# kyshu11027/financial-chatbot-llm

Hardware: AMD Instinct MI355X
Metric: chat turns/sec + p50 TTFT, Llama-3-8B RAG agent at 1/2/4/8 MI355X (higher is better)
Workload: dtype bf16

## Files before the change

financial_chatbot_llm_amd/csrc/kernels/gemm_splitk.hip:

```cpp
#include "common.h"

#include <utility>

typedef __attribute__((address_space(3))) void lds_void_t;
typedef __attribute__((address_space(1))) const void gbl_void_t;

namespace {

template <int N>
__device__ __forceinline__ void vmcnt_barrier() {
  static_assert(N >= 0 && N < 64, "vmcnt range");
  asm volatile("s_waitcnt vmcnt(%0)\n\ts_barrier" ::"n"(N) : "memory");
}

union Frag {
  uint4 u;
  bf16x8 v;
};

enum { SK_SLAB = 0, SK_SILU = 1, SK_BF16 = 2, SK_SAMPLE = 3, SK_SAMPLE_LP = 4 };

struct SkSample {
  const float* temps;
  const unsigned long long* seeds;
  float* pv;
  int* pi;
  int pstride, voff, vvalid;
};

__device__ __forceinline__ int xswz(int r, int c) { return c ^ (r & 7) ^ ((r >> 3) & 1); }

template <int NF, int MT, int KB = 150, int MAXB = 8, int BKM = 1>
struct Ring {
  static constexpr int SBYTES = (NF + MT) * 2 * 1024 * BKM;
  static constexpr int LOADS = (2 * NF + 2 * MT) / 4 * BKM;
  static constexpr int BY_LDS = KB * 1024 / SBYTES;
  static constexpr int BY_VM = 63 / LOADS + 2;
  static constexpr int CAP = MAXB / BKM > 3 ? MAXB / BKM : 3;
  static constexpr int NBUF = BY_LDS < CAP ? (BY_LDS < BY_VM ? BY_LDS : BY_VM) : (CAP < BY_VM ? CAP : BY_VM);
};

template <class F, int... U>
__device__ __forceinline__ void static_for_impl(F&& f, std::integer_sequence<int, U...>) {
  (f(std::integral_constant<int, U>{}), ...);
}
template <int N, class F>
__device__ __forceinline__ void static_for(F&& f) {
  static_for_impl(f, std::make_integer_sequence<int, N>{});
}

template <int LOADS, int MAXY>
__device__ __forceinline__ void wait_stage(int younger) {
  if constexpr (MAXY <= 0) {
    vmcnt_barrier<0>();
  } else {
    if (younger >= MAXY) vmcnt_barrier<MAXY * LOADS>();
    else wait_stage<LOADS, MAXY - 1>(younger);
  }
}

template <int FW, int TW, int WBYTES, bool WROW>
__device__ __forceinline__ void stage_mma(const char* __restrict__ base, f32x4 (&acc)[FW][TW], int wa, int wb,
                                          int lane, int g, int col) {
#pragma unroll
  for (int kk = 0; kk < 2; ++kk) {
    Frag wf[FW], xf[TW];
#pragma unroll
    for (int f = 0; f < FW; ++f) {
      if constexpr (WROW) {
        const int r = (wa * FW + f) * 16 + col;
        wf[f].u = *reinterpret_cast<const uint4*>(base + r * 128 + xswz(r, 4 * kk + g) * 16);
      } else {
        wf[f].u = *reinterpret_cast<const uint4*>(base + ((wa * FW + f) * 2 + kk) * 1024 + lane * 16);
      }
    }
#pragma unroll
    for (int t = 0; t < TW; ++t) {
      const int r = (wb * TW + t) * 16 + col;
      xf[t].u = *reinterpret_cast<const uint4*>(base + WBYTES + r * 128 + xswz(r, 4 * kk + g) * 16);
    }
#pragma unroll
    for (int f = 0; f < FW; ++f)
#pragma unroll
      for (int t = 0; t < TW; ++t)
        acc[f][t] = __builtin_amdgcn_mfma_f32_16x16x32_bf16(wf[f].v, xf[t].v, acc[f][t], 0, 0, 0);
  }
}

template <int NF, int MT, int WA, int EPI = SK_SLAB, bool WROW = false, int RKB = 150, int MAXB = 8, int BKM = 1>
__global__ void __launch_bounds__(256, 1) splitk_gemm_kernel(const bf16* __restrict__ X, int ldx,
                                                             const bf16* __restrict__ Wt, int K,
                                                             float* __restrict__ P, int M, int N, int S,
                                                             bf16* __restrict__ Y = nullptr, int ldy = 0,
                                                             SkSample sa = SkSample{}) {
  constexpr bool SILU = EPI == SK_SILU;
  constexpr int WB = 4 / WA;
  constexpr int FW = NF / WA;
  constexpr int TW = MT / WB;
  static_assert(NF % WA == 0 && MT % WB == 0, "wave split");
  static_assert(!SILU || FW % 2 == 0, "SiLU epilogue needs (gate, up) row-group pairs per wave");
  constexpr int NBUF = Ring<NF, MT, RKB, MAXB, BKM>::NBUF;
  static_assert(NBUF >= 3, "ring too shallow");
  constexpr int WBYTES = NF * 2 * 1024;
  constexpr int XBYTES = MT * 2 * 1024;
  constexpr int SBYTES = WBYTES + XBYTES;
  constexpr int PIECES = (2 * NF + 2 * MT);
  static_assert(PIECES % 4 == 0, "pieces must split evenly over 4 waves");
  constexpr int LOADS = PIECES / 4;
  constexpr int SLOT = BKM * SBYTES;
  __shared__ __attribute__((aligned(1024))) char smem[NBUF * SLOT];

  const int lane = threadIdx.x & 63, w = threadIdx.x >> 6, g = lane >> 4, col = lane & 15;
  const int s = blockIdx.x % S, tile = blockIdx.x / S;
  const int Mtot = M, m0 = blockIdx.y * 16 * MT;
  M = min(Mtot - m0, 16 * MT);
  X += (long)m0 * ldx;
  if constexpr (EPI == SK_SILU || EPI == SK_BF16) Y += (long)m0 * ldy;
  PENNY_DASSERT(M > 0 && ((EPI != SK_SAMPLE && EPI != SK_SAMPLE_LP) || gridDim.y == 1));
  PENNY_DASSERT((tile + 1) * 16 * NF <= N && K % (64 * BKM * S) == 0);
  const int n0 = tile * 16 * NF;
  const int kc = K / S, k0 = s * kc;
  const int nst = kc / (64 * BKM);
  const int ksteps = K / 32;
  const int wa = w / WB, wb = w % WB;

  const char* src[LOADS];
  int dst[LOADS];
  long step[LOADS];
#pragma unroll
  for (int i = 0; i < LOADS; ++i) {
    const int q = w * LOADS + i;
    if (q < 2 * NF && WROW) {
      const int r = q * 8 + (lane >> 3);
      const int c = xswz(r, lane & 7);
      src[i] = reinterpret_cast<const char*>(Wt + (long)(n0 + r) * K + k0 + 8 * c);
      step[i] = 128;
      dst[i] = q * 1024;
    } else if (q < 2 * NF) {
      const int f = q >> 1, kk = q & 1;
      src[i] = reinterpret_cast<const char*>(Wt) +
               (((long)(n0 / 16 + f) * ksteps + k0 / 32 + kk) * 64 + lane) * 16;
      step[i] = 2 * 1024;
      dst[i] = (f * 2 + kk) * 1024;
    } else {
      const int xp = q - 2 * NF;
      const int r = xp * 8 + (lane >> 3);
      const int c = xswz(r, lane & 7);
      const int row = min(r, M - 1);
      src[i] = reinterpret_cast<const char*>(X + (long)row * ldx + k0 + 8 * c);
      step[i] = 128;
      dst[i] = WBYTES + xp * 1024;
    }
  }
  auto stage = [&](int j) {
    char* base = smem + (j % NBUF) * SLOT;
#pragma unroll
    for (int i = 0; i < LOADS; ++i)
#pragma unroll
      for (int u = 0; u < BKM; ++u)
        __builtin_amdgcn_global_load_lds((gbl_void_t*)(src[i] + (j * BKM + u) * step[i]),
                                         (lds_void_t*)(base + u * SBYTES + dst[i]), 16, 0, 0);
  };

  f32x4 acc[FW][TW];
#pragma unroll
  for (int f = 0; f < FW; ++f)
#pragma unroll
    for (int t = 0; t < TW; ++t) acc[f][t] = f32x4{0.f, 0.f, 0.f, 0.f};

#pragma unroll
  for (int j = 0; j < NBUF - 1; ++j)
    if (j < nst) stage(j);

  for (int j = 0; j < nst; ++j) {
    wait_stage<LOADS * BKM, NBUF - 2>(min(NBUF - 2, nst - 1 - j));
    if (j + NBUF - 1 < nst) stage(j + NBUF - 1);
#pragma unroll
    for (int u = 0; u < BKM; ++u)
      stage_mma<FW, TW, WBYTES, WROW>(smem + (j % NBUF) * SLOT + u * SBYTES, acc, wa, wb, lane, g, col);
  }

  if constexpr (SILU) {
#pragma unroll
    for (int t = 0; t < TW; ++t) {
      const int m = (wb * TW + t) * 16 + col;
      if (m >= M) continue;
#pragma unroll
      for (int f = 0; f < FW; f += 2) {
        const int G = n0 / 16 + wa * FW + f;
        bf16x4 o;
#pragma unroll
        for (int r = 0; r < 4; ++r) {
          const float gt = (float)(bf16)acc[f][t][r], up = (float)(bf16)acc[f + 1][t][r];
          o[r] = (bf16)((float)(bf16)(gt / (1.f + __expf(-gt))) * up);
        }
        *reinterpret_cast<bf16x4*>(Y + (long)m * ldy + (G >> 1) * 16 + 4 * g) = o;
      }
    }
    return;
  }
  if constexpr (EPI == SK_BF16) {
#pragma unroll
    for (int t = 0; t < TW; ++t) {
      const int m = (wb * TW + t) * 16 + col;
      if (m >= M) continue;
#pragma unroll
      for (int f = 0; f < FW; ++f) {
        bf16x4 o;
#pragma unroll
        for (int r = 0; r < 4; ++r) o[r] = (bf16)acc[f][t][r];
        *reinterpret_cast<bf16x4*>(Y + (long)m * ldy + n0 + (wa * FW + f) * 16 + 4 * g) = o;
      }
    }
    return;
  }
  if constexpr (EPI == SK_SAMPLE) {
#pragma unroll
    for (int t = 0; t < TW; ++t) {
      const int m = (wb * TW + t) * 16 + col;
      if (m >= M) continue;
      const float temp = sa.temps[m];
      const bool greedy = !(temp > 0.f);
      const float inv_t = greedy ? 1.f : 1.f / temp;
      const unsigned long long seed = sa.seeds[m];
      float bv = -INFINITY;
      int bi = 0x7fffffff;
#pragma unroll
      for (int f = 0; f < FW; ++f)
#pragma unroll
        for (int r = 0; r < 4; ++r) {
          const int loc = n0 + (wa * FW + f) * 16 + 4 * g + r, idx = sa.voff + loc;
          float v = (float)(bf16)acc[f][t][r];
          if (!greedy) v = v * inv_t + gumbel_noise(seed, idx);
          if (loc >= sa.vvalid) v = -INFINITY;
          better(bv, bi, v, idx);
        }
#pragma unroll
      for (int o = 16; o < 64; o <<= 1) {
        const float ov = __shfl_xor(bv, o, 64);
        const int oi = __shfl_xor(bi, o, 64);
        better(bv, bi, ov, oi);
      }
      if (g == 0) {
        const long slot = (long)m * sa.pstride + tile * WA + wa;
        sa.pv[slot] = bv;
        sa.pi[slot] = bi;
      }
    }
    return;
  }
  if constexpr (EPI == SK_SAMPLE_LP) {
    const long plane = (long)Mtot * sa.pstride;
    float* pl = sa.pv + 2 * plane;
    float* pm = pl + plane;
    float* pe = pm + plane;
#pragma unroll
    for (int t = 0; t < TW; ++t) {
      const int m = (wb * TW + t) * 16 + col;
      if (m >= M) continue;
      const float temp = sa.temps[m];
      const bool greedy = !(temp > 0.f);
      const float inv_t = greedy ? 1.f : 1.f / temp;
      const unsigned long long seed = sa.seeds[m];
      const int loc0 = n0 + wa * FW * 16 + 4 * g;
      float bv = -INFINITY, bl = -INFINITY, mx = -INFINITY;
      int bi = 0x7fffffff;
#pragma unroll
      for (int f = 0; f < FW; ++f)
#pragma unroll
        for (int r = 0; r < 4; ++r) {
          const int loc = loc0 + f * 16 + r, idx = sa.voff + loc;
          const float l = (float)(bf16)acc[f][t][r];
          float v = l;
          if (!greedy) v = v * inv_t + gumbel_noise(seed, idx);
          if (loc >= sa.vvalid) v = -INFINITY;
          else mx = fmaxf(mx, l);
          better_lp(bv, bi, bl, v, idx, l);
        }
#pragma unroll
      for (int o = 16; o < 64; o <<= 1) {
        const float ov = __shfl_xor(bv, o, 64);
        const int oi = __shfl_xor(bi, o, 64);
        const float ol = __shfl_xor(bl, o, 64);
        better_lp(bv, bi, bl, ov, oi, ol);
        mx = fmaxf(mx, __shfl_xor(mx, o, 64));
      }
      float se = 0.f;
#pragma unroll
      for (int f = 0; f < FW; ++f)
#pragma unroll
        for (int r = 0; r < 4; ++r)
          if (loc0 + f * 16 + r < sa.vvalid) se += __expf((float)(bf16)acc[f][t][r] - mx);
#pragma unroll
      for (int o = 16; o < 64; o <<= 1) se += __shfl_xor(se, o, 64);
      if (g == 0) {
        const long slot = (long)m * sa.pstride + tile * WA + wa;
        sa.pv[slot] = bv;
        sa.pi[slot] = bi;
        pl[slot] = bl;
        pm[slot] = mx;
        pe[slot] = se;
      }
    }
    return;
  }
  float* ps = P + (long)s * Mtot * N + (long)m0 * N;
#pragma unroll
  for (int t = 0; t < TW; ++t) {
    const int m = (wb * TW + t) * 16 + col;
    if (m >= M) continue;
#pragma unroll
    for (int f = 0; f < FW; ++f) {
      const int n = n0 + (wa * FW + f) * 16 + 4 * g;
      *reinterpret_cast<f32x4*>(ps + (long)m * N + n) = acc[f][t];
    }
  }
}

__global__ void __launch_bounds__(256) splitk_reduce_kernel(const float* __restrict__ P, int S, int M, int N,
                                                            bf16* __restrict__ Y, int ldy,
                                                            const bf16* __restrict__ R, int ldr) {
  const long i8 = (long)blockIdx.x * 256 + threadIdx.x;
  const long total8 = (long)M * N / 8;
  if (i8 >= total8) return;
  const int m = (int)(i8 / (N / 8));
  const int n = (int)(i8 % (N / 8)) * 8;
  float o[8];
  {
    const f32x4* p = reinterpret_cast<const f32x4*>(P + (long)m * N + n);
    const f32x4 a = p[0], b = p[1];
#pragma unroll
    for (int j = 0; j < 4; ++j) o[j] = a[j], o[4 + j] = b[j];
  }
  for (int s = 1; s < S; ++s) {
    const f32x4* p = reinterpret_cast<const f32x4*>(P + ((long)s * M + m) * N + n);
    const f32x4 a = p[0], b = p[1];
#pragma unroll
    for (int j = 0; j < 4; ++j) o[j] += a[j], o[4 + j] += b[j];
  }
  if (R) {
    float r[8];
    unpack8(*reinterpret_cast<const uint4*>(R + (long)m * ldr + n), r);
#pragma unroll
    for (int j = 0; j < 8; ++j) o[j] = (float)(bf16)o[j] + r[j];
  }
  *reinterpret_cast<uint4*>(Y + (long)m * ldy + n) = pack8(o);
}

template <int NF, int MT, int RKB, int MAXB>
constexpr bool pair_fits() {
  return Ring<NF, MT, RKB, MAXB, 2>::NBUF >= 3;
}

constexpr int wave_split(int nf, int mt) { return nf >= 6 || mt <= 2 || (mt > 4 && mt <= 6) ? 2 : 1; }

template <int NF, int MT, int EPI, int MAXB, int WA = wave_split(NF, MT), class... A>
int launch_any(int wrow, bool pair_ok, dim3 grid, hipStream_t st, A... args) {
  const bool rm = wrow & 1;
  if constexpr (pair_fits<NF, MT, 150, MAXB>()) {
    if ((wrow & 2) && pair_ok) {
      if (rm) hipLaunchKernelGGL((splitk_gemm_kernel<NF, MT, WA, EPI, true, 150, MAXB, 2>), grid, dim3(256), 0, st, args...);
      else hipLaunchKernelGGL((splitk_gemm_kernel<NF, MT, WA, EPI, false, 150, MAXB, 2>), grid, dim3(256), 0, st, args...);
      return (int)hipGetLastError();
    }
  }
  if (rm) hipLaunchKernelGGL((splitk_gemm_kernel<NF, MT, WA, EPI, true, 150, MAXB>), grid, dim3(256), 0, st, args...);
  else hipLaunchKernelGGL((splitk_gemm_kernel<NF, MT, WA, EPI, false, 150, MAXB>), grid, dim3(256), 0, st, args...);
  return (int)hipGetLastError();
}

template <int NF, int MT>
int launch(const void* X, int ldx, const void* Wt, int K, float* P, int M, int N, int S, int wrow, hipStream_t st) {
  return launch_any<NF, MT, SK_SLAB, 8>(wrow, (K / S) % 128 == 0, dim3((N / (16 * NF)) * S, (M + 16 * MT - 1) / (16 * MT)), st, (const bf16*)X,
                                            ldx, (const bf16*)Wt, K, P, M, N, S, (bf16*)nullptr, 0, SkSample{});
}

template <int NF, int MT>
int launch_silu(const void* X, int ldx, const void* Wt, int K, void* Y, int ldy, int M, int N, int wrow,
                hipStream_t st) {
  constexpr int WA = NF == 2 ? 1 : wave_split(NF, MT);
  return launch_any<NF, MT, SK_SILU, NF == 2 ? 16 : 8, WA>(wrow, K % 128 == 0, dim3(N / (16 * NF), (M + 16 * MT - 1) / (16 * MT)), st, (const bf16*)X,
                                                          ldx, (const bf16*)Wt, K, (float*)nullptr, M, N, 1, (bf16*)Y,
                                                          ldy, SkSample{});
}

template <int NF, int MT>
int launch_bf16(const void* X, int ldx, const void* Wt, int K, void* Y, int ldy, int M, int N, int wrow,
                hipStream_t st) {
  return launch_any<NF, MT, SK_BF16, 16>(wrow, K % 128 == 0, dim3(N / (16 * NF), (M + 16 * MT - 1) / (16 * MT)), st, (const bf16*)X, ldx,
                                             (const bf16*)Wt, K, (float*)nullptr, M, N, 1, (bf16*)Y, ldy, SkSample{});
}

template <int NF, int MT, int EPI>
int launch_sample(const void* X, int ldx, const void* Wt, int K, int M, int N, int wrow, int ring2, const SkSample& sa,
                  hipStream_t st) {
  constexpr int WA = wave_split(NF, MT);
  const dim3 grid(N / (16 * NF)), block(256);
#define SK_SAMPLE_LAUNCH(WROW_, KB_)                                                                               \
  hipLaunchKernelGGL((splitk_gemm_kernel<NF, MT, WA, EPI, WROW_, KB_, 16>), grid, block, 0, st, (const bf16*)X, ldx, \
// ... 39 lines not shown
  return (int)hipErrorInvalidValue;
}

PENNY_API int penny_splitk_gemm(const void* X, int ldx, const void* Wt, int K, void* P, int M, int N, int S, int nf,
                                int wrow, hipStream_t stream) {
  if (M <= 0) return 0;
  if (M > (1 << 20) || S < 1 || K % (64 * S) || ldx % 8 || (nf != 2 && nf != 4 && nf != 6 && nf != 8) || N % (16 * nf))
    return (int)hipErrorInvalidValue;
  const int mt = min((M + 15) / 16, 16);
  float* p = static_cast<float*>(P);
#define SK_CASE(MT_)                                                             \
  if (mt <= MT_) {                                                               \
    if (nf == 2) return launch<2, MT_>(X, ldx, Wt, K, p, M, N, S, wrow, stream); \
    if (nf == 4) return launch<4, MT_>(X, ldx, Wt, K, p, M, N, S, wrow, stream); \
    if (nf == 6) return launch<6, MT_>(X, ldx, Wt, K, p, M, N, S, wrow, stream); \
    return launch<8, MT_>(X, ldx, Wt, K, p, M, N, S, wrow, stream);              \
  }
  SK_CASE(2) SK_CASE(4) SK_CASE(6) SK_CASE(8) SK_CASE(12) SK_CASE(16)
#undef SK_CASE
  return (int)hipErrorInvalidValue;
}

__global__ void __launch_bounds__(256) splitk_reduce_silu_kernel(const float* __restrict__ P, int S, int M, int N,
                                                                 bf16* __restrict__ Y, int ldy) {
  const int F = N / 2;
  const long i8 = (long)blockIdx.x * 256 + threadIdx.x;
  const long total8 = (long)M * F / 8;
  if (i8 >= total8) return;
  const int m = (int)(i8 / (F / 8));
  const int f = (int)(i8 % (F / 8)) * 8;
  const int ng = (f >> 4) * 32 + (f & 15);
  float gt[8], up[8];
#pragma unroll
  for (int j = 0; j < 8; ++j) gt[j] = up[j] = 0.f;
  for (int s = 0; s < S; ++s) {
    const f32x4* pg = reinterpret_cast<const f32x4*>(P + ((long)s * M + m) * N + ng);
    const f32x4* pu = reinterpret_cast<const f32x4*>(P + ((long)s * M + m) * N + ng + 16);
    const f32x4 g0 = pg[0], g1 = pg[1], u0 = pu[0], u1 = pu[1];
#pragma unroll
    for (int j = 0; j < 4; ++j) gt[j] += g0[j], gt[4 + j] += g1[j], up[j] += u0[j], up[4 + j] += u1[j];
  }
  float o[8];
#pragma unroll
  for (int j = 0; j < 8; ++j) {
    const float gb = (float)(bf16)gt[j], ub = (float)(bf16)up[j];
    o[j] = (float)(bf16)(gb / (1.f + __expf(-gb))) * ub;
  }
  *reinterpret_cast<uint4*>(Y + (long)m * ldy + f) = pack8(o);
}

PENNY_API int penny_splitk_reduce_silu(const void* P, int S, int M, int N, void* Y, int ldy, hipStream_t stream) {
  if (M <= 0) return 0;
  if (N % 32 || ldy % 8 || S < 1) return (int)hipErrorInvalidValue;
  const long total8 = (long)M * (N / 2) / 8;
  hipLaunchKernelGGL(splitk_reduce_silu_kernel, dim3((unsigned)((total8 + 255) / 256)), dim3(256), 0, stream,
                     (const float*)P, S, M, N, (bf16*)Y, ldy);
  return (int)hipGetLastError();
}

PENNY_API int penny_splitk_reduce(const void* P, int S, int M, int N, void* Y, int ldy, const void* R, int ldr,
                                  hipStream_t stream) {
  if (M <= 0) return 0;
  if (N % 8 || ldy % 8 || (R && ldr % 8)) return (int)hipErrorInvalidValue;
  const long total8 = (long)M * N / 8;
  hipLaunchKernelGGL(splitk_reduce_kernel, dim3((unsigned)((total8 + 255) / 256)), dim3(256), 0, stream,
                     (const float*)P, S, M, N, (bf16*)Y, ldy, (const bf16*)R, ldr);
  return (int)hipGetLastError();
}

PENNY_API int penny_splitk_gemm_bf16(const void* X, int ldx, const void* Wt, int K, void* Y, int ldy, int M, int N,
                                     int nf, int wrow, hipStream_t stream) {
  if (M <= 0) return 0;
  if (M > (1 << 20) || K % 64 || ldx % 8 || ldy % 4 || (nf != 2 && nf != 4 && nf != 8) || N % (16 * nf))
    return (int)hipErrorInvalidValue;
  const int mt = min((M + 15) / 16, 16);
#define BF_CASE(MT_)                                                                    \
  if (mt <= MT_) {                                                                      \
    if (nf == 2) return launch_bf16<2, MT_>(X, ldx, Wt, K, Y, ldy, M, N, wrow, stream); \
    if (nf == 4) return launch_bf16<4, MT_>(X, ldx, Wt, K, Y, ldy, M, N, wrow, stream); \
    return launch_bf16<8, MT_>(X, ldx, Wt, K, Y, ldy, M, N, wrow, stream);              \
  }
  BF_CASE(2) BF_CASE(4) BF_CASE(6) BF_CASE(8) BF_CASE(12) BF_CASE(16)
#undef BF_CASE
  return (int)hipErrorInvalidValue;
}

extern "C" int penny_lm_sample_logprob_final(const float* pv, const int* pi, const float* pl, const float* pm,
                                             const float* ps, int P, int M, int* out, float* logprob,
                                             hipStream_t stream);

template <int EPI, class Merge>
static int stream_sample(const void* X, int ldx, const void* W, int K, int M, int Vpad, int vvalid, int voff,
                         const float* temps, const unsigned long long* seeds, void* workspace, int nf, int wrow,
                         int ring2, hipStream_t stream, Merge merge) {
  if (M > 128 || (nf != 4 && nf != 8) || Vpad % (16 * nf) || vvalid <= 0 || vvalid > Vpad || voff < 0 || K % 64 ||
      ldx % 8 || !temps || !seeds || !workspace)
    return (int)hipErrorInvalidValue;
  const int tiles = Vpad / (16 * nf), mt = (M + 15) / 16;
  const int pstride = tiles * wave_split(nf, mt);
  float* pv = static_cast<float*>(workspace);
  int* pi = reinterpret_cast<int*>(pv + (long)M * pstride);
  const SkSample sa{temps, seeds, pv, pi, pstride, voff, vvalid};
  int rc;
#define LS_CASE(MT_)                                                                            \
  if (mt <= MT_) {                                                                              \
    if (nf == 4) rc = launch_sample<4, MT_, EPI>(X, ldx, W, K, M, Vpad, wrow, ring2, sa, stream); \
    else rc = launch_sample<8, MT_, EPI>(X, ldx, W, K, M, Vpad, wrow, ring2, sa, stream);         \
  } else
  LS_CASE(2) LS_CASE(4) LS_CASE(6) LS_CASE(8)
  return (int)hipErrorInvalidValue;
#undef LS_CASE
  if (rc) return rc;
  return merge(pv, pi, pstride);
}

PENNY_API int penny_lm_head_stream_sample(const void* X, int ldx, const void* W, int K, int M, int Vpad, int vvalid,
                                          int voff, const float* temps, const unsigned long long* seeds,
                                          void* workspace, int* out, int* pairs, int nf, int wrow, int ring2,
                                          hipStream_t stream) {
  if (M <= 0) return 0;
  if (!out && !pairs) return (int)hipErrorInvalidValue;
  return stream_sample<SK_SAMPLE>(X, ldx, W, K, M, Vpad, vvalid, voff, temps, seeds, workspace, nf, wrow, ring2,
                                  stream, [=](const float* pv, const int* pi, int P) {
                                    return penny_lm_sample_final(pv, pi, P, M, out, pairs, stream);
                                  });
}

PENNY_API int penny_lm_head_stream_sample_logprob(const void* X, int ldx, const void* W, int K, int M, int Vpad,
                                                  int vvalid, int voff, const float* temps,
                                                  const unsigned long long* seeds, void* workspace, int* out,
                                                  float* logprob, int nf, int wrow, int ring2, hipStream_t stream) {
  if (M <= 0) return 0;
  if (!out || !logprob) return (int)hipErrorInvalidValue;
  return stream_sample<SK_SAMPLE_LP>(X, ldx, W, K, M, Vpad, vvalid, voff, temps, seeds, workspace, nf, wrow, ring2,
                                     stream, [=](const float* pv, const int* pi, int P) {
                                       const long plane = (long)M * P;
                                       return penny_lm_sample_logprob_final(pv, pi, pv + 2 * plane, pv + 3 * plane,
                                                                            pv + 4 * plane, P, M, out, logprob,
                                                                            stream);
                                     });
}
```

financial_chatbot_llm_amd/ops/_native.py:

```python
from __future__ import annotations

import ctypes
import os
import threading
from typing import Optional

import torch

_LOCK = threading.Lock()
_LIB: Optional[ctypes.CDLL] = None
_ERR: Optional[str] = None

c_int, c_long, c_float, c_void_p = ctypes.c_int, ctypes.c_long, ctypes.c_float, ctypes.c_void_p
P = c_void_p

_SIGS = {
    "penny_rmsnorm": [P, P, P, P, c_int, c_int, c_float, c_int, P],
    "penny_rmsnorm_slabs": [P, c_int, P, P, P, c_int, c_int, c_float, c_int, P],
    "penny_layernorm": [P, P, P, P, P, c_int, c_int, c_float, c_int, P],
    "penny_silu_mul": [P, P, c_int, c_int, c_int, P],
    "penny_skinny_gemm": [P, c_int, P, c_int, P, c_int, P, c_int, c_int, c_int, c_int, c_int, c_int, P],
    "penny_splitk_gemm": [P, c_int, P, c_int, P, c_int, c_int, c_int, c_int, c_int, P],
    "penny_splitk_reduce": [P, c_int, c_int, c_int, P, c_int, P, c_int, P],
    "penny_splitk_gemm_bf16": [P, c_int, P, c_int, P, c_int, c_int, c_int, c_int, c_int, P],
    "penny_lm_head_stream_sample": [P, c_int, P, c_int, c_int, c_int, c_int, c_int, P, P, P, P, P, c_int, c_int,
                                    c_int, P],
    "penny_lm_sample_final": [P, P, c_int, c_int, P, P, P],
    "penny_gateup_silu_gemm": [P, c_int, P, c_int, P, c_int, c_int, c_int, c_int, c_int, P],
    "penny_gemm_prefill": [P, c_int, P, c_int, P, c_int, P, c_int, c_int, c_int, c_int, c_int,
                           P, c_long, P, c_int, c_int, P],
    "penny_gemm_prefill_wt": [P, c_int, P, c_int, P, c_int, P, c_int, c_int, c_int, c_int, c_int,
                              P, c_long, P, c_int, c_int, P],
    "penny_gemm_prefill_qkv_rope": [P, c_int, P, c_int, c_int, P, P, P, P, P, P, c_int, c_int,
                                    c_float, P, c_long, P, c_int, c_int, P],
    "penny_gemm_mid_variant": [c_int],
    "penny_gemm_mid": [P, c_int, P, c_int, P, c_int, P, c_int, c_int, c_int, c_int, c_int, P],
    "penny_gemm_prefill_ablate": [P, c_int, P, c_int, P, c_int, c_int, c_int, c_int, P],
    "penny_moe_gemm_prefill_fp8": [P, c_int, P, P, P, P, P, P, P, c_int, c_int, c_int, c_int, c_int, c_int, P],
    "penny_probe_mfma_scale": [P, P, P, P, P, c_int, P],
    "penny_moe_gemm_prefill_fp8_mx": [P, c_int, P, P, P, P, P, P, P, c_int, c_int, c_int, c_int, c_int, c_int, P,
                                      c_int, P],
    "penny_gelu": [P, c_long, P],
    "penny_embedding": [P, P, P, c_int, c_int, c_int, c_int, P],
    "penny_rope_qk": [P, P, P, P, c_int, c_int, c_int, c_int, P],
    "penny_rope_kv_write": [P, P, P, P, P, P, P, c_int, c_int, c_int, c_int, c_int, P],
    "penny_rope_kv_write_slabs": [P, c_int, P, P, P, P, P, P, c_int, c_int, c_int, c_int, c_int, P],
    "penny_rope_kv_write_fp8": [P, P, P, P, P, P, P, P, c_int, c_int, c_int, c_int, c_int, P],
    "penny_rope_kv_write_slabs_fp8": [P, c_int, P, P, P, P, P, P, P, c_int, c_int, c_int, c_int, c_int, P],
    "penny_kv_dequant_fp8": [P, P, P, c_long, c_int, c_int, P],
    "penny_attention_decode_fp8": [P, P, P, P, P, P, P, P, P, c_int, c_int, c_int, c_int, c_int, c_int, c_int,
                                   c_float, c_int, P, c_int, c_int, P, P],
    "penny_attention_prefill_fp8": [P, P, P, P, P, P, P, c_int, c_int, c_int, c_int, c_int, c_int, c_float, c_int, P,
                                    P, c_int, P, P],
    "penny_attention_prefill_lean_fp8": [P, P, P, P, P, P, P, c_int, c_int, c_int, c_int, c_float, c_int, P, P,
                                         c_int, P, c_int, P, P, P, P],
    "penny_attention_prefill": [P, P, P, P, P, P, P, c_int, c_int, c_int, c_int, c_int, c_int, c_float, c_int, P, P,
                                c_int, P],
    "penny_attention_prefill_variant": [c_int],
    "penny_gemm_prefill_set_group": [c_int],
    "penny_attention_prefill_lean": [P, P, P, P, P, P, P, c_int, c_int, c_int, c_int, c_float, c_int, P, P, c_int, P,
                                     c_int, P, P, P],
    "penny_splitk_reduce_silu": [P, c_int, c_int, c_int, P, c_int, P],
    "penny_attention_decode": [P, P, P, P, P, P, P, P, P, c_int, c_int, c_int, c_int, c_int, c_int, c_int, c_int,
                               c_float, c_int, P, c_int, c_int, P],
    "penny_sample": [P, c_int, c_long, P, P, P, P, P, P, c_int, c_int, P],
    "penny_sample_fsm": [P, c_int, c_long, P, P, P, P, P, P, c_int, c_int, P, P, P, c_int, c_int, P, P, P, c_int, P,
                         c_int, P],
    "penny_fsm_build_masks": [P, P, P, P, P, c_int, c_int, c_int, c_int, c_int, c_int, P],
    "penny_pen_reset": [P, c_int, c_int, c_int, c_int, P, c_int, P],
    "penny_pen_add": [P, c_int, c_int, c_int, P, c_int, P],
    "penny_pen_apply": [P, c_int, c_long, P, P, P, P, P, P, c_int, c_int, P, c_int, c_int, P],
    "penny_lm_head_sample": [P, c_int, P, c_int, c_int, c_int, P, P, P, P, P],
    "penny_lm_head_sample_shard": [P, c_int, P, c_int, c_int, c_int, c_int, c_int, P, P, P, P, P],
    "penny_lm_head_logprob": [P, c_int, P, c_int, c_int, c_int, c_int, c_int, P, P, P, P, P],
    "penny_lm_head_sample_logprob": [P, c_int, P, c_int, c_int, c_int, c_int, c_int, P, P, P, P, P, P],
    "penny_lm_head_stream_sample_logprob": [P, c_int, P, c_int, c_int, c_int, c_int, c_int, P, P, P, P, P, c_int,
                                            c_int, c_int, P],
    "penny_lm_sample_logprob_final": [P, P, P, P, P, c_int, c_int, P, P, P],
    "penny_token_logprob": [P, c_int, c_long, P, P, c_int, c_int, P],
    "penny_sample_shard": [P, c_int, c_long, P, P, P, P, c_int, c_int, c_int, P],
    "penny_topk_topp_threshold": [P, c_int, c_long, P, P, P, P, c_int, c_int, P],
    "penny_moe_route": [P, c_int, c_int, c_int, P, P, P, P, P],
    "penny_moe_route_quant": [P, c_int, P, c_int, c_int, c_int, c_int, P, P, P, P, P, P, P, P, P],
    "penny_quant_rows_fp8": [P, c_int, c_int, c_int, P, P, P],
    "penny_silu_quant_rows_fp8": [P, c_int, c_int, P, P, P],
    "penny_moe_gemm_fp8": [P, P, P, P, P, P, P, P, c_int, c_int, c_int, c_int, c_int, P],
    "penny_moe_combine": [P, P, c_int, c_int, c_int, P, P],
    "penny_moe_combine_weighted": [P, P, P, c_int, c_int, c_int, P, P],
    "penny_filtered_topk": [P, P, P, c_long, c_int, P, P, P, P, c_int, c_int, P, P, P, c_int, P, P, P, P],
}


def lib_path() -> str:
    if os.environ.get("PENNY_KERNEL_LIB"):
        return os.environ["PENNY_KERNEL_LIB"]
    from .._build import kernel_lib
    return kernel_lib(os.environ.get("PENNY_KERNEL_DEBUG") == "1")


def load(build_if_missing: bool = True) -> ctypes.CDLL:
    global _LIB, _ERR
    if _LIB is not None:
        return _LIB
    with _LOCK:
        if _LIB is not None:
            return _LIB
        path = lib_path()
# ... 50 lines not shown
```

financial_chatbot_llm_amd/ops/gemm.py:

```python
from __future__ import annotations

import os
from typing import Dict, List, Optional, Tuple, Union

import torch
import torch.nn.functional as F

from . import _native as N
from .activation import silu_mul

EPI = {None: 0, "silu": 1, "residual": 2}
MAX_SKINNY_M = 64
TUNING: Dict[Tuple[int, int], Tuple[int, int]] = {(6144, 4096): (2, 4), (4096, 4096): (1, 4)}
SKINNY_MAX_M: Dict[Tuple[int, int], int] = {(6144, 4096): 16, (4096, 4096): 32}


def _config(N_: int, K: int, epilogue: Optional[str]) -> Tuple[int, int]:
    if (N_, K) in TUNING:
        return TUNING[(N_, K)]
    ntf = 2
    wgs = N_ // (16 * ntf)
    nw = 8 if wgs < 512 else 4
    if K % (nw * 128):
        nw = 4 if K % 512 == 0 else 1
    return ntf, nw


def tile_weight(w: torch.Tensor) -> torch.Tensor:
    N_, K = w.shape
    assert N_ % 16 == 0 and K % 32 == 0
    return w.view(N_ // 16, 16, K // 32, 4, 8).permute(0, 2, 3, 1, 4).reshape(N_ // 16, K // 32, 64, 8).contiguous()


def skinny_ok(x: torch.Tensor, w: torch.Tensor, epilogue: Optional[str] = None,
              wt: Optional[torch.Tensor] = None) -> bool:
    M, K = x.shape
    N_ = w.shape[0]
    if wt is None or not N.use_native(x) or M > MAX_SKINNY_M or os.environ.get("PENNY_SKINNY", "1") == "0":
        return False
    if M > SKINNY_MAX_M.get((N_, K), MAX_SKINNY_M if (N_, K) in TUNING else 0):
        return False
    ntf, nw = _config(N_, K, epilogue)
    return N_ % (16 * ntf) == 0 and K % (nw * 128) == 0 and x.stride(1) == 1 and w.is_contiguous()


def linear(x: torch.Tensor, w: torch.Tensor, epilogue: Optional[str] = None,
           residual: Optional[torch.Tensor] = None, wt: Optional[torch.Tensor] = None,
           slabs: bool = False, fuse_residual: Optional[torch.Tensor] = None) -> Union[torch.Tensor, "Slabs",
                                                                                     "ResidualSum"]:
    M, K = x.shape
    N_ = w.shape[0]
    if M > 256 and prefill_ok(x, w) and epilogue in (None, "silu", "residual"):
        fr = fuse_residual is not None and epilogue is None and residual is None
        c = prefill_choice(M, N_, K, epilogue, slabs and residual is None, fused_residual=fr)
        if c.startswith("K"):
            return splitk_bf16(x, w, N_, int(c[1:]))
        if c == "R":
            prefill_gemm(x, w, "residual", residual=fuse_residual, out=fuse_residual)
            return ResidualSum(fuse_residual)
        if c == "hip":
            return prefill_gemm(x, w, epilogue, residual=residual)
        if c.startswith("S"):
            return Slabs(prefill_gemm(x, w, "slabs", int(c[1:])))
        if c.startswith("M"):
            return mid_linear(x, w, int(c[1:]), epilogue, slabs and residual is None, residual)
    src = wt if wt is not None else (w if w.is_contiguous() else None)
    rowmajor = wt is None
    if slabs and src is not None and epilogue is None and residual is None:
        cfg = splitk_config(M, N_, K) if N.use_native(x) and x.stride(1) == 1 and x.stride(0) % 8 == 0 else None
        if cfg is not None:
            return Slabs(splitk_partials(x, src, N_, *cfg, rowmajor=rowmajor))
    if not slabs and epilogue is None and residual is None and N.use_native(x) and x.stride(1) == 1 \
            and x.stride(0) % 8 == 0:
        cfg = bf16_config(M, N_, K)
        if cfg is not None:
            S, nf, rm = cfg
            rm = rm or wt is None
            ww = w if rm else wt
            if S == 1:
                return splitk_bf16(x, ww, N_, nf, rowmajor=rm)
            return splitk_reduce(splitk_partials(x, ww, N_, S, nf, rowmajor=rm))
    if epilogue == "silu" and src is not None and residual is None:
        ok = N.use_native(x) and x.stride(1) == 1 and x.stride(0) % 8 == 0
        nf = gateup_config(M, N_, K) if ok else None
        if nf is not None:
            return gateup_silu(x, src, N_, nf, rowmajor=rowmajor)
        cfg = gateup_splitk_config(M, N_, K) if ok else None
        if cfg is not None and (cfg[2] or not rowmajor):
            S, nf, rm = cfg
            return gateup_splitk(x, w if rm else src, N_, S, nf, rowmajor=rm)
    if skinny_ok(x, w, epilogue, wt):
        ntf, nw = _config(N_, K, epilogue)
        out_n = N_ // 2 if epilogue == "silu" else N_
        y = torch.empty((M, out_n), dtype=x.dtype, device=x.device)
        N.call("penny_skinny_gemm", N.ptr(x), x.stride(0), N.ptr(wt), K, N.ptr(y), out_n, N.ptr(residual),
               residual.stride(0) if residual is not None else 0, M, N_, EPI[epilogue], ntf, nw, N.stream())
        return y
    y = F.linear(x, w)
    if epilogue == "silu":
        return silu_mul(y, interleave16=True)
    if epilogue == "residual":
        return (y.float() + residual.float()).to(y.dtype) if not N.use_native(y) else y.add_(residual)
    return y


def interleave16(gate: torch.Tensor, up: torch.Tensor) -> torch.Tensor:
    Fr, H = gate.shape
    return torch.stack([gate.view(Fr // 16, 16, H), up.view(Fr // 16, 16, H)], dim=1).reshape(2 * Fr, H)


TUNING_DIR = os.path.join(os.path.dirname(os.path.dirname(os.path.abspath(__file__))), "tuning")
_LOADED_TUNING: Optional[str] = None


def tuning_file(model: str, tp: int = 1) -> str:
    suffix = "" if tp == 1 else f"_tp{tp}"
    return os.path.join(TUNING_DIR, f"gemm_{model}{suffix}_mi355x.csv")


def load_gemm_tuning(model: str, tp: int = 1) -> Optional[str]:
    global _LOADED_TUNING
    path = tuning_file(model, tp)
    if os.environ.get("PENNY_GEMM_TUNING", "1") != "1" or not os.path.exists(path) or not torch.cuda.is_available():
        return None
    if _LOADED_TUNING == path:
        return path
    tun = torch.cuda.tunable
    tun.tuning_enable(False)
    tun.record_untuned_enable(False)
    if not tun.read_file(path):
        return None
    tun.enable(True)
    _LOADED_TUNING = path
    return path


SPLITK: Dict[Tuple[int, int], List[Tuple[int, int, int]]] = {
    (6144, 4096): [(256, 4, 6)],
    (4096, 4096): [(32, 4, 2), (256, 4, 4)],
    (4096, 14336): [(16, 8, 8), (32, 4, 4), (256, 8, 8)],
    (8192, 28672): [(8, 8, 2), (256, 4, 8)],
    (8192, 8192): [(32, 8, 2), (128, 8, 8), (256, 4, 8)],
    (10240, 8192): [(32, 8, 2), (256, 2, 8)],
    (1280, 8192): [(256, 8, 4)],
}
TILE_FREE = {(8192, 28672), (8192, 8192), (1280, 8192), (10240, 8192)}


DECODE_BF16: Dict[Tuple[int, int], List[Tuple[int, int, int, bool]]] = {
    (8192, 1024): [(32, 1, 4, True), (256, 1, 2, True)],
    (8192, 3584): [(64, 1, 2, True), (96, 2, 4, True), (128, 4, 8, True), (256, 2, 4, True)],
}


def bf16_config(M: int, N_: int, K: int) -> Optional[Tuple[int, int, bool]]:
    mode = os.environ.get("PENNY_SPLITK", "1")
    if mode == "0" or M > 256 or K % 64:
        return None
    for max_m, S, nf, rm in DECODE_BF16.get((N_, K), ()):
        if M <= max_m:
            return (S, nf, rm) if nf > 0 and K % (64 * S) == 0 else None
    if mode == "force":
        for nf in (2, 4):
            if N_ % (16 * nf) == 0:
                return 1, nf, True
    return None
# ... 46 lines not shown
        if M <= max_m:
            return gateup_silu(x, wt, N_, nf) if S == 1 else gateup_splitk(x, wt, N_, S, nf)
    return gateup_silu(x, wt, N_, 8)


def uses_tiled_weight(N_: int, K: int) -> bool:
    if (N_, K) in TUNING or (N_, K) in TILED_ONLY:
        return True
    if DECODE_WEIGHTS == "rowmajor" or (N_, K) in TILE_FREE:
        return False
    if os.environ.get("PENNY_SPLITK", "1") == "force":
        return True
    return (N_, K) in SPLITK or (N_, K) in GATEUP or any(not e[4] for e in GATEUP_SPLITK.get((N_, K), ()))


def splitk_config(M: int, N_: int, K: int) -> Optional[Tuple[int, int]]:
    mode = os.environ.get("PENNY_SPLITK", "1")
    if mode == "0" or M > 256:
        return None
    for max_m, S, nf in SPLITK.get((N_, K), ()):
        if M <= max_m:
            return (S, nf) if S > 0 else None
    if mode == "force":
        nf = 4 if N_ % 64 == 0 else 2
        for S in (4, 2, 1):
            if K % (64 * S) == 0 and N_ % (16 * nf) == 0:
                return S, nf
    return None


GATEUP: Dict[Tuple[int, int], List[Tuple[int, int, int]]] = {
    (28672, 4096): [(2, 256, 8)],
}


def gateup_config(M: int, N_: int, K: int) -> Optional[int]:
    mode = os.environ.get("PENNY_GATEUP", "1")
    if mode == "0" or M > 256 or K % 64:
        return None
    for lo, hi, nf in GATEUP.get((N_, K), ()):
        if lo <= M <= hi:
            return nf
    if mode == "force":
        return 8 if N_ % 128 == 0 else (4 if N_ % 64 == 0 else None)
    return None


def gateup_silu(x: torch.Tensor, wt: torch.Tensor, N_: int, nf: int,
                out: Optional[torch.Tensor] = None, rowmajor: bool = False) -> torch.Tensor:
    M, K = x.shape
    if not N.use_native(x):
        return silu_mul(F.linear(x, wt if rowmajor else untile_weight(wt)), interleave16=True)
    y = out if out is not None else torch.empty((M, N_ // 2), dtype=x.dtype, device=x.device)
    N.call("penny_gateup_silu_gemm", N.ptr(x), x.stride(0), N.ptr(wt), K, N.ptr(y), y.stride(0), M, N_, nf,
           _wrow(rowmajor, M, N_, K), N.stream())
    return y


GATEUP_SPLITK: Dict[Tuple[int, int], List[Tuple[int, int, int, int, bool]]] = {
    (7168, 8192): [(1, 64, 2, 4, False), (65, 256, 4, 8, False)],
    (57344, 8192): [(1, 1, 8, 2, True), (2, 16, 4, 2, True)],
    (28672, 4096): [(1, 1, 4, 2, False)],
}


def gateup_splitk_config(M: int, N_: int, K: int) -> Optional[Tuple[int, int, bool]]:
    if os.environ.get("PENNY_GATEUP", "1") == "0" or M > 256:
        return None
    for lo, hi, S, nf, rm in GATEUP_SPLITK.get((N_, K), ()):
        if lo <= M <= hi and K % (64 * S) == 0 and N_ % (32 * nf) == 0:
            return S, nf, rm
    return None


def gateup_splitk(x: torch.Tensor, w: torch.Tensor, N_: int, S: int, nf: int, rowmajor: bool = False,
                  slabs: Optional[torch.Tensor] = None, out: Optional[torch.Tensor] = None) -> torch.Tensor:
    M, K = x.shape
    P = splitk_partials(x, w, N_, S, nf, out=slabs, rowmajor=rowmajor)
    if not N.use_native(x):
        g = P.sum(0).to(torch.bfloat16)
        return silu_mul(g, interleave16=True)
    y = out if out is not None else torch.empty((M, N_ // 2), dtype=x.dtype, device=x.device)
    N.call("penny_splitk_reduce_silu", N.ptr(P), S, M, N_, N.ptr(y), y.stride(0), N.stream())
    return y


class ResidualSum:

    __slots__ = ("t",)

    def __init__(self, t: torch.Tensor):
        self.t = t

    @property
    def shape(self):
        return self.t.shape


class Slabs:

    __slots__ = ("P",)

    def __init__(self, P: torch.Tensor):
        self.P = P

    @property
    def shape(self) -> Tuple[int, int]:
        return (self.P.shape[1], self.P.shape[2])

    def materialize(self) -> torch.Tensor:
        return splitk_reduce(self.P)


def splitk_partials(x: torch.Tensor, wt: torch.Tensor, N_: int, S: int, nf: int,
                    out: Optional[torch.Tensor] = None, rowmajor: bool = False) -> torch.Tensor:
    M, K = x.shape
    if not N.use_native(x):
        w = (wt if rowmajor else untile_weight(wt)).float()
        xs = x.float().view(M, S, K // S).transpose(0, 1)
        return torch.einsum("smk,snk->smn", xs, w.view(N_, S, K // S).transpose(0, 1))
    P = out if out is not None else torch.empty((S, M, N_), dtype=torch.float32, device=x.device)
    N.call("penny_splitk_gemm", N.ptr(x), x.stride(0), N.ptr(wt), K, N.ptr(P), M, N_, S, nf,
           _wrow(rowmajor, M, N_, K), N.stream())
    return P


def splitk_reduce(P: torch.Tensor, residual: Optional[torch.Tensor] = None,
                  out: Optional[torch.Tensor] = None) -> torch.Tensor:
    S, M, N_ = P.shape
    if not N.use_native(P):
        y = P.sum(0).to(torch.bfloat16)
        return y if residual is None else (y.float() + residual.float()).to(torch.bfloat16)
    y = out if out is not None else torch.empty((M, N_), dtype=torch.bfloat16, device=P.device)
    N.call("penny_splitk_reduce", N.ptr(P), S, M, N_, N.ptr(y), y.stride(0), N.ptr(residual),
           residual.stride(0) if residual is not None else 0, N.stream())
    return y


PREFILL_EPI = {None: 0, "silu": 1, "slabs": 2, "residual": 3, "bias": 5, "bias_gelu": 6}


PREFILL_POLICY: Dict[Tuple[int, int], List[Tuple[int, str]]] = {
    (6144, 4096): [(1 << 30, "fused")],
    (4096, 4096): [(384, "M4"), (1024, "M2"), (2048, "S2"), (1 << 30, "R")],
    (28672, 4096): [(1 << 30, "hip")],
    (4096, 14336): [(512, "M4"), (1024, "S4"), (1280, "hip"), (2048, "S2"), (1 << 30, "R")],
    (10240, 8192): [(384, "M2"), (768, "S2"), (1 << 30, "fused")],
    (8192, 8192): [(512, "S4"), (1024, "S2"), (1 << 30, "R")],
    (57344, 8192): [(1 << 30, "hip")],
    (8192, 28672): [(512, "S4"), (768, "S2"), (1024, "hip"), (1536, "S4"), (1 << 30, "R")],
    (1280, 8192): [(1024, "M8"), (1536, "M4"), (3072, "S4"), (1 << 30, "S2")],
    (8192, 1024): [(1536, "M1"), (1 << 30, "hip")],
    (7168, 8192): [(384, "M4"), (512, "M2"), (1 << 30, "hip")],
    (8192, 3584): [(384, "M2"), (1024, "M1"), (1 << 30, "hip")],
}


def _default_choice(M: int, N_: int, K: int, epilogue: Optional[str]) -> str:
    tiles = -(-M // 256) * (N_ // 256)
    return "hip" if tiles >= 224 or (epilogue in ("silu", "bias_gelu") and tiles >= 112) else "lib"


def prefill_choice(M: int, N_: int, K: int, epilogue: Optional[str] = None, slabs: bool = False,
                   fused_residual: bool = False) -> str:
    if os.environ.get("PENNY_PREFILL_GEMM", "1") == "0":
        return "lib"
# ... 204 lines not shown
```

Baseline: 42.36.

## Add register-ring streaming GEMM kernel for mid-batch decode 4096x4096 projections

Adds a new stream_gemm kernel in which each wave holds a ring of weight fragments in registers, loaded directly from global memory with manual vmcnt waits. Activations are double-buffered through LDS via global_load_lds, overlapping weight streaming with MFMA work. The kernel is routed in for 4096x4096 GEMMs at batch sizes 97-256 for the slab and bf16 paths, and the epilogues are factored into a shared store_tiles helper. The inline asm waits and the hand-built schedule add correctness risk and raise register pressure.

```diff
diff --git a/financial_chatbot_llm_amd/csrc/kernels/gemm_splitk.hip b/financial_chatbot_llm_amd/csrc/kernels/gemm_splitk.hip
--- a/financial_chatbot_llm_amd/csrc/kernels/gemm_splitk.hip
+++ b/financial_chatbot_llm_amd/csrc/kernels/gemm_splitk.hip
@@ -84,6 +84,53 @@
 #pragma unroll
       for (int t = 0; t < TW; ++t)
         acc[f][t] = __builtin_amdgcn_mfma_f32_16x16x32_bf16(wf[f].v, xf[t].v, acc[f][t], 0, 0, 0);
+  }
+}
+
+template <int EPI, int FW, int TW>
+__device__ __forceinline__ void store_tiles(const f32x4 (&acc)[FW][TW], int rg0, int t0, int n0, int M, int N,
+                                            float* __restrict__ ps, bf16* __restrict__ Y, int ldy, int g, int col) {
+  if constexpr (EPI == SK_SILU) {
+#pragma unroll
+    for (int t = 0; t < TW; ++t) {
+      const int m = (t0 + t) * 16 + col;
+      if (m >= M) continue;
+#pragma unroll
+      for (int f = 0; f < FW; f += 2) {
+        const int G = n0 / 16 + rg0 + f;
+        bf16x4 o;
+#pragma unroll
+        for (int r = 0; r < 4; ++r) {
+          const float gt = (float)(bf16)acc[f][t][r], up = (float)(bf16)acc[f + 1][t][r];
+          o[r] = (bf16)((float)(bf16)(gt / (1.f + __expf(-gt))) * up);
+        }
+        *reinterpret_cast<bf16x4*>(Y + (long)m * ldy + (G >> 1) * 16 + 4 * g) = o;
+      }
+    }
+  } else if constexpr (EPI == SK_BF16) {
+#pragma unroll
+    for (int t = 0; t < TW; ++t) {
+      const int m = (t0 + t) * 16 + col;
+      if (m >= M) continue;
+#pragma unroll
+      for (int f = 0; f < FW; ++f) {
+        bf16x4 o;
+#pragma unroll
+        for (int r = 0; r < 4; ++r) o[r] = (bf16)acc[f][t][r];
+        *reinterpret_cast<bf16x4*>(Y + (long)m * ldy + n0 + (rg0 + f) * 16 + 4 * g) = o;
+      }
+    }
+  } else {
+#pragma unroll
+    for (int t = 0; t < TW; ++t) {
+      const int m = (t0 + t) * 16 + col;
+      if (m >= M) continue;
+#pragma unroll
+      for (int f = 0; f < FW; ++f) {
+        const int n = n0 + (rg0 + f) * 16 + 4 * g;
+        *reinterpret_cast<f32x4*>(ps + (long)m * N + n) = acc[f][t];
+      }
+    }
   }
 }
 
@@ -180,38 +227,8 @@
       stage_mma<FW, TW, WBYTES, WROW>(smem + (j % NBUF) * SLOT + u * SBYTES, acc, wa, wb, lane, g, col);
   }
 
-  if constexpr (SILU) {
-#pragma unroll
-    for (int t = 0; t < TW; ++t) {
-      const int m = (wb * TW + t) * 16 + col;
-      if (m >= M) continue;
-#pragma unroll
-      for (int f = 0; f < FW; f += 2) {
-        const int G = n0 / 16 + wa * FW + f;
-        bf16x4 o;
-#pragma unroll
-        for (int r = 0; r < 4; ++r) {
-          const float gt = (float)(bf16)acc[f][t][r], up = (float)(bf16)acc[f + 1][t][r];
-          o[r] = (bf16)((float)(bf16)(gt / (1.f + __expf(-gt))) * up);
-        }
-        *reinterpret_cast<bf16x4*>(Y + (long)m * ldy + (G >> 1) * 16 + 4 * g) = o;
-      }
-    }
-    return;
-  }
-  if constexpr (EPI == SK_BF16) {
-#pragma unroll
-    for (int t = 0; t < TW; ++t) {
-      const int m = (wb * TW + t) * 16 + col;
-      if (m >= M) continue;
-#pragma unroll
-      for (int f = 0; f < FW; ++f) {
-        bf16x4 o;
-#pragma unroll
-        for (int r = 0; r < 4; ++r) o[r] = (bf16)acc[f][t][r];
-        *reinterpret_cast<bf16x4*>(Y + (long)m * ldy + n0 + (wa * FW + f) * 16 + 4 * g) = o;
-      }
-    }
+  if constexpr (EPI == SK_SILU || EPI == SK_BF16) {
+    store_tiles<EPI, FW, TW>(acc, wa * FW, wb * TW, n0, M, N, nullptr, Y, ldy, g, col);
     return;
   }
   if constexpr (EPI == SK_SAMPLE) {
@@ -304,17 +321,131 @@
     }
     return;
   }
-  float* ps = P + (long)s * Mtot * N + (long)m0 * N;
-#pragma unroll
-  for (int t = 0; t < TW; ++t) {
-    const int m = (wb * TW + t) * 16 + col;
-    if (m >= M) continue;
-#pragma unroll
-    for (int f = 0; f < FW; ++f) {
-      const int n = n0 + (wa * FW + f) * 16 + 4 * g;
-      *reinterpret_cast<f32x4*>(ps + (long)m * N + n) = acc[f][t];
-    }
-  }
+  store_tiles<SK_SLAB, FW, TW>(acc, wa * FW, wb * TW, n0, M, N, P + (long)s * Mtot * N + (long)m0 * N, nullptr, 0, g, col);
+}
+
+constexpr int XS_K = 256;
+
+__device__ __forceinline__ void wload(Frag& d, const char* p) {
+  bf16x8 t;
+  asm volatile("global_load_dwordx4 %0, %1, off" : "=v"(t) : "v"(p));
+  d.v = t;
+}
+template <int VM, int FW>
+__device__ __forceinline__ void ring_wait(Frag (&slot)[FW]) {
+  static_assert(VM >= 0 && VM < 64 && (FW == 1 || FW == 2), "vmcnt range");
+  bf16x8 a = slot[0].v, b = slot[FW - 1].v;
+  if constexpr (FW == 1) asm volatile("s_waitcnt vmcnt(%1)" : "+v"(a) : "n"(VM));
+  else asm volatile("s_waitcnt vmcnt(%2)" : "+v"(a), "+v"(b) : "n"(VM));
+  slot[0].v = a;
+  if constexpr (FW == 2) slot[1].v = b;
+}
+
+template <int FW, int MT, int RING, bool LAST>
+__device__ __forceinline__ void stream_stage(const char* __restrict__ xb, f32x4 (&acc)[FW][MT], Frag (&ring)[RING][FW],
+                                             const char* const (&wsrc)[FW], int nx0, int g, int col) {
+  constexpr int XBYTES = MT * 2 * 1024;
+  Frag xf[2][MT];
+  auto read_x = [&](int u) {
+#pragma unroll
+    for (int t = 0; t < MT; ++t) {
+      const int r = t * 16 + col;
+      xf[u & 1][t].u = *reinterpret_cast<const uint4*>(xb + (u / 2) * XBYTES + r * 128 + xswz(r, 4 * (u & 1) + g) * 16);
+    }
+  };
+  read_x(0);
+  static_for<RING>([&](auto uc) {
+    constexpr int u = decltype(uc)::value;
+    if constexpr (u + 1 < RING) read_x(u + 1);
+    ring_wait<LAST ? (RING - 1 - u) * FW : (RING - 1) * FW + 2 * MT, FW>(ring[u]);
+#pragma unroll
+    for (int f = 0; f < FW; ++f)
+#pragma unroll
+      for (int t = 0; t < MT; ++t)
+        acc[f][t] = __builtin_amdgcn_mfma_f32_16x16x32_bf16(ring[u][f].v, xf[u & 1][t].v, acc[f][t], 0, 0, 0);
+    if constexpr (!LAST) {
+#pragma unroll
+      for (int f = 0; f < FW; ++f) wload(ring[u][f], wsrc[f] + (long)(nx0 + u) * 1024);
+    }
+    __builtin_amdgcn_sched_barrier(0);
+  });
+}
+
+template <int NF, int MT, int EPI>
+__global__ void __launch_bounds__(256, 1) stream_gemm_kernel(const bf16* __restrict__ X, int ldx,
+                                                             const bf16* __restrict__ Wt, int K,
+                                                             float* __restrict__ P, int M, int N, int S,
+                                                             bf16* __restrict__ Y, int ldy) {
+  static_assert(NF % 4 == 0 && MT % 2 == 0, "wave split");
+  static_assert(EPI == SK_SLAB || EPI == SK_BF16 || (EPI == SK_SILU && NF % 8 == 0), "epilogue");
+  constexpr int FW = NF / 4;
+  constexpr int RING = XS_K / 32;
+  constexpr int XBYTES = MT * 2 * 1024;
+  constexpr int NBLK = XS_K / 64;
+  constexpr int XL = MT / 2;
+  __shared__ __attribute__((aligned(1024))) char smem[2 * NBLK * XBYTES];
+
+  const int lane = threadIdx.x & 63, w = threadIdx.x >> 6, g = lane >> 4, col = lane & 15;
+  const int s = blockIdx.x % S, tile = blockIdx.x / S;
+  const int Mtot = M, m0 = blockIdx.y * 16 * MT;
+  M = min(Mtot - m0, 16 * MT);
+  X += (long)m0 * ldx;
+  if constexpr (EPI != SK_SLAB) Y += (long)m0 * ldy;
+  PENNY_DASSERT(M > 0 && (tile + 1) * 16 * NF <= N && K % (XS_K * S) == 0);
+  const int n0 = tile * 16 * NF;
+  const int kc = K / S, k0 = s * kc;
+  const int nks = kc / 32, ksteps = K / 32, nss = kc / XS_K;
+
+  const char* xsrc[XL];
+  int xdst[XL];
+#pragma unroll
+  for (int i = 0; i < XL; ++i) {
+    const int xp = w * XL + i;
+    const int r = xp * 8 + (lane >> 3);
+    const int c = xswz(r, lane & 7);
+    xsrc[i] = reinterpret_cast<const char*>(X + (long)min(r, M - 1) * ldx + k0 + 8 * c);
+    xdst[i] = xp * 1024;
+  }
+  auto fill = [&](int ss) {
+#pragma unroll
+    for (int b = 0; b < NBLK; ++b)
+#pragma unroll
+      for (int i = 0; i < XL; ++i)
+        __builtin_amdgcn_global_load_lds((gbl_void_t*)(xsrc[i] + (ss * XS_K + b * 64) * 2),
+                                         (lds_void_t*)(smem + ((ss & 1) * NBLK + b) * XBYTES + xdst[i]), 16, 0, 0);
+  };
+  const char* wsrc[FW];
+#pragma unroll
+  for (int f = 0; f < FW; ++f)
+    wsrc[f] = reinterpret_cast<const char*>(Wt) + (((long)(n0 / 16 + w * FW + f) * ksteps + k0 / 32) * 64 + lane) * 16;
+
+  fill(0);
+  Frag ring[RING][FW];
+#pragma unroll
+  for (int u = 0; u < RING; ++u)
+#pragma unroll
+    for (int f = 0; f < FW; ++f) wload(ring[u][f], wsrc[f] + u * 1024);
+
+  f32x4 acc[FW][MT];
+#pragma unroll
+  for (int f = 0; f < FW; ++f)
+#pragma unroll
+    for (int t = 0; t < MT; ++t) acc[f][t] = f32x4{0.f, 0.f, 0.f, 0.f};
+
+  constexpr int VM = RING * FW;
+  for (int ss = 0; ss < nss - 1; ++ss) {
+    __builtin_amdgcn_s_waitcnt((VM & 15) | ((VM >> 4) << 14) | 0x0F70);
+    __builtin_amdgcn_s_barrier();
+    fill(ss + 1);
+    stream_stage<FW, MT, RING, false>(smem + (ss & 1) * NBLK * XBYTES, acc, ring, wsrc, (ss + 1) * RING, g, col);
+  }
+  __builtin_amdgcn_s_waitcnt((VM & 15) | ((VM >> 4) << 14) | 0x0F70);
+  __builtin_amdgcn_s_barrier();
+  stream_stage<FW, MT, RING, true>(smem + ((nss - 1) & 1) * NBLK * XBYTES, acc, ring, wsrc, 0, g, col);
+  asm volatile("s_waitcnt vmcnt(0)" ::: "memory");
+  __builtin_amdgcn_sched_barrier(0);
+  store_tiles<EPI, FW, MT>(acc, w * FW, 0, n0, M, N, EPI == SK_SLAB ? P + (long)s * Mtot * N + (long)m0 * N : nullptr, Y,
+                           ldy, g, col);
 }
 
 __global__ void __launch_bounds__(256) splitk_reduce_kernel(const float* __restrict__ P, int S, int M, int N,
@@ -520,6 +651,31 @@
   }
   BF_CASE(2) BF_CASE(4) BF_CASE(6) BF_CASE(8) BF_CASE(12) BF_CASE(16)
 #undef BF_CASE
+  return (int)hipErrorInvalidValue;
+}
+
+PENNY_API int penny_decode_stream_gemm(const void* X, int ldx, const void* Wt, int K, void* P, void* Y, int ldy, int M,
+                                       int N, int S, int nf, int epi, hipStream_t stream) {
+  if (M <= 0) return 0;
+  if (M > (1 << 20) || S < 1 || K % (256 * S) || ldx % 8 || (nf != 4 && nf != 8) || N % (16 * nf) || epi < 0 || epi > 2 ||
+      (epi == SK_SLAB ? !P : (!Y || S != 1 || ldy % 4)) || (epi == SK_SILU && nf != 8))
+    return (int)hipErrorInvalidValue;
+  const int mt = min((M + 15) / 16, 8);
+#define ST_LAUNCH(NF_, MT_, EPI_)                                                                                \
+  hipLaunchKernelGGL((stream_gemm_kernel<NF_, MT_, EPI_>), dim3((N / (16 * NF_)) * S, (M + 16 * MT_ - 1) / (16 * MT_)), \
+                     dim3(256), 0, stream, (const bf16*)X, ldx, (const bf16*)Wt, K, (float*)P, M, N, S, (bf16*)Y, ldy)
+#define ST_CASE(MT_)                                       \
+  if (mt <= MT_) {                                         \
+    if (epi == SK_SILU) ST_LAUNCH(8, MT_, SK_SILU);        \
+    else if (epi == SK_BF16 && nf == 4) ST_LAUNCH(4, MT_, SK_BF16); \
+    else if (epi == SK_BF16) ST_LAUNCH(8, MT_, SK_BF16);   \
+    else if (nf == 4) ST_LAUNCH(4, MT_, SK_SLAB);          \
+    else ST_LAUNCH(8, MT_, SK_SLAB);                       \
+    return (int)hipGetLastError();                         \
+  }
+  ST_CASE(4) ST_CASE(6) ST_CASE(8)
+#undef ST_CASE
+#undef ST_LAUNCH
   return (int)hipErrorInvalidValue;
 }
 
diff --git a/financial_chatbot_llm_amd/ops/_native.py b/financial_chatbot_llm_amd/ops/_native.py
--- a/financial_chatbot_llm_amd/ops/_native.py
+++ b/financial_chatbot_llm_amd/ops/_native.py
@@ -23,6 +23,7 @@
     "penny_splitk_gemm": [P, c_int, P, c_int, P, c_int, c_int, c_int, c_int, c_int, P],
     "penny_splitk_reduce": [P, c_int, c_int, c_int, P, c_int, P, c_int, P],
     "penny_splitk_gemm_bf16": [P, c_int, P, c_int, P, c_int, c_int, c_int, c_int, c_int, P],
+    "penny_decode_stream_gemm": [P, c_int, P, c_int, P, P, c_int, c_int, c_int, c_int, c_int, c_int, P],
     "penny_lm_head_stream_sample": [P, c_int, P, c_int, c_int, c_int, c_int, c_int, P, P, P, P, P, c_int, c_int,
                                     c_int, P],
     "penny_lm_sample_final": [P, P, c_int, c_int, P, P, P],
diff --git a/financial_chatbot_llm_amd/ops/gemm.py b/financial_chatbot_llm_amd/ops/gemm.py
--- a/financial_chatbot_llm_amd/ops/gemm.py
+++ b/financial_chatbot_llm_amd/ops/gemm.py
@@ -67,12 +67,20 @@
     src = wt if wt is not None else (w if w.is_contiguous() else None)
     rowmajor = wt is None
     if slabs and src is not None and epilogue is None and residual is None:
-        cfg = splitk_config(M, N_, K) if N.use_native(x) and x.stride(1) == 1 and x.stride(0) % 8 == 0 else None
+        ok = N.use_native(x) and x.stride(1) == 1 and x.stride(0) % 8 == 0
+        cfg = stream_config(M, N_, K) if ok and not rowmajor else None
+        if cfg is not None:
+            return Slabs(stream_gemm(x, wt, N_, *cfg))
+        cfg = splitk_config(M, N_, K) if ok else None
         if cfg is not None:
             return Slabs(splitk_partials(x, src, N_, *cfg, rowmajor=rowmajor))
     if not slabs and epilogue is None and residual is None and N.use_native(x) and x.stride(1) == 1 \
             and x.stride(0) % 8 == 0:
         cfg = bf16_config(M, N_, K)
+        sc = stream_config(M, N_, K) if cfg is not None and wt is not None else None
+        if sc is not None:
+            S, nf = sc
+            return stream_gemm(x, wt, N_, 1, nf, "bf16") if S == 1 else splitk_reduce(stream_gemm(x, wt, N_, S, nf))
         if cfg is not None:
             S, nf, rm = cfg
             rm = rm or wt is None
@@ -82,6 +90,9 @@
             return splitk_reduce(splitk_partials(x, ww, N_, S, nf, rowmajor=rm))
     if epilogue == "silu" and src is not None and residual is None:
         ok = N.use_native(x) and x.stride(1) == 1 and x.stride(0) % 8 == 0
+        cfg = stream_config(M, N_, K, silu=True) if ok and not rowmajor else None
+        if cfg is not None:
+            return stream_gemm(x, wt, N_, 1, 8, "silu")
         nf = gateup_config(M, N_, K) if ok else None
         if nf is not None:
             return gateup_silu(x, src, N_, nf, rowmajor=rowmajor)
@@ -294,6 +305,52 @@
         return silu_mul(g, interleave16=True)
     y = out if out is not None else torch.empty((M, N_ // 2), dtype=x.dtype, device=x.device)
     N.call("penny_splitk_reduce_silu", N.ptr(P), S, M, N_, N.ptr(y), y.stride(0), N.stream())
+    return y
+
+
+DECODE_STREAM: Dict[Tuple[int, int], List[Tuple[int, int, int, int]]] = {
+    (4096, 4096): [(97, 128, 4, 4), (193, 256, 4, 8)],
+}
+STREAM_EPI = {None: 0, "silu": 1, "bf16": 2}
+
+
+def stream_ok(N_: int, K: int, S: int, nf: int, silu: bool = False) -> bool:
+    return (S >= 1 and nf in (4, 8) and N_ % (16 * nf) == 0 and K % (256 * S) == 0
+            and (not silu or (S == 1 and nf == 8)))
+
+
+def stream_config(M: int, N_: int, K: int, silu: bool = False) -> Optional[Tuple[int, int]]:
+    mode = os.environ.get("PENNY_DECODE_STREAM", "1")
+    if mode == "0" or M > 256:
+        return None
+    for lo, hi, S, nf in DECODE_STREAM.get((N_, K), ()):
+        if lo <= M <= hi:
+            return (S, nf) if stream_ok(N_, K, S, nf, silu) else None
+    if mode == "force":
+        for S, nf in ((1, 8),) if silu else ((4, 8), (4, 4), (2, 4), (1, 4)):
+            if stream_ok(N_, K, S, nf, silu):
+                return S, nf
+    return None
+
+
+def stream_gemm(x: torch.Tensor, wt: torch.Tensor, N_: int, S: int, nf: int, epilogue: Optional[str] = None,
+                out: Optional[torch.Tensor] = None) -> torch.Tensor:
+    M, K = x.shape
+    if not N.use_native(x):
+        if epilogue == "silu":
+            return gateup_silu(x, wt, N_, nf, out=out)
+        return splitk_partials(x, wt, N_, S, nf, out=out) if epilogue is None else splitk_bf16(x, wt, N_, nf, False, out)
+    if not stream_ok(N_, K, S, nf, epilogue == "silu") or (epilogue is not None and S != 1):
+        raise ValueError(f"decode stream GEMM cannot serve N={N_} K={K} S={S} nf={nf} epilogue={epilogue}")
+    if epilogue is None:
+        y = out if out is not None else torch.empty((S, M, N_), dtype=torch.float32, device=x.device)
+        args = (N.ptr(y), None, 0)
+    else:
+        cols = N_ // 2 if epilogue == "silu" else N_
+        y = out if out is not None else torch.empty((M, cols), dtype=x.dtype, device=x.device)
+        args = (None, N.ptr(y), y.stride(0))
+    N.call("penny_decode_stream_gemm", N.ptr(x), x.stride(0), N.ptr(wt), K, *args, M, N_, S, nf,
+           STREAM_EPI[epilogue], N.stream())
     return y
 
 
```

After: 42.23. About the same (-0.3%).
